# StephenNG59/ICP-symm

Hardware: AMD Instinct MI355X
Metric: icp_iterations_per_sec (higher is better)
Workload: dtype f32

## Files before the change

icp-symm_amd/csrc/engine.cpp:

```cpp
#include "engine_internal.h"
#include "robust_loss.h"
#include <limits>

void read_switches(Switches &w)
{
    auto flag = [](const char *n) { return std::getenv(n) != nullptr; };
    auto num = [](const char *n, long def) { const char *e = std::getenv(n); return e ? std::atol(e) : def; };
    auto tri = [](const char *n) { const char *e = std::getenv(n); return e ? (e[0] == '1' ? 1 : 0) : -1; };
    w.allow_any_arch = flag("SYMMICP_ALLOW_ANY_ARCH");
    w.debug_host = flag("SYMMICP_DEBUG_HOST");
    w.debug_counters = flag("SYMMICP_DEBUG_COUNTERS");
    if (const char *e = std::getenv("SYMMICP_DEBUG_TRACE")) w.debug_trace = e;
    if (const char *e = std::getenv("SYMMICP_GRID_PPC")) w.grid_ppc = std::atof(e);
    w.grid_maxlevel = (int)num("SYMMICP_GRID_MAXLEVEL", kMortonBits);
    w.grid_level = (int)num("SYMMICP_GRID_LEVEL", -1);
    if (const char *e = std::getenv("SYMMICP_FIRST_PASS")) w.first_pass = (e[0] == 'p') ? 1 : 0;
    w.oct_leaf = (int)num("SYMMICP_OCT_LEAF", 0);
    if (const char *e = std::getenv("SYMMICP_PACKET_ORDER")) w.packet_order = e[0] != '0';
    if (const char *e = std::getenv("SYMMICP_PACKET_JUMP")) w.packet_jump = (float)std::atof(e);
    w.packet_key_bits = (int)num("SYMMICP_PACKET_KEY_BITS", 16);
    w.packet_chunk = (uint32_t)num("SYMMICP_PACKET_CHUNK", 0);
    w.packet_lds_pad = (uint32_t)num("SYMMICP_PACKET_LDS_PAD", 0);
    w.packet_waves = (uint32_t)num("SYMMICP_PACKET_WAVES", 0);
    w.packet_front_cap = (uint32_t)num("SYMMICP_PACKET_FRONT_CAP", 0);
    if (const char *e = std::getenv("SYMMICP_HOOD_FRAC")) w.hood_frac = std::atof(e);
    w.no_hood = flag("SYMMICP_NO_NEIGHBOURHOOD");
    w.no_cert = flag("SYMMICP_NO_CERT");
    w.walk_full_grid = flag("SYMMICP_WALK_FULL_GRID");
    { const char *e = std::getenv("SYMMICP_HOST_LOOP"); w.host_loop = e && e[0] == '1'; }
    w.no_loop_stragglers = flag("SYMMICP_NO_LOOP_STRAGGLERS");
    w.force_comm = flag("SYMMICP_FORCE_COMM");
    if (const char *e = std::getenv("SYMMICP_PACKET_COST_KEY")) w.packet_cost_key = e[0] != '0';
    w.budget_walk = tri("SYMMICP_BUDGET_WALK");
    w.optimistic = tri("SYMMICP_OPTIMISTIC");
    w.compact = tri("SYMMICP_COMPACT");
    w.cert_pass = (int)num("SYMMICP_CERT_PASS", 1);
    w.cert_head = (int)num("SYMMICP_CERT_HEAD", 4);
    w.pass_blocks = (int)num("SYMMICP_PASS_BLOCKS", 2048);
    w.id_blocks = (int)num("SYMMICP_ID_BLOCKS", 2048);
    w.acc_blocks = (int)num("SYMMICP_ACC_BLOCKS", 512);
    w.fused_blocks = (int)num("SYMMICP_FUSED_BLOCKS", 512);
    w.compact_blocks = (int)num("SYMMICP_COMPACT_BLOCKS", 1280);
    w.feature_nn_splits = (int)num("SYMMICP_FEATURE_NN_SPLITS", 0);
    w.feature_nn_queries = (int)num("SYMMICP_FEATURE_NN_QUERIES", 0);
    w.plane_score = (int)num("SYMMICP_PLANE_SCORE", 0);
    w.tune.wave_mode_max =(uint32_t)num("SYMMICP_WAVE_MODE_MAX", 20000);
    w.tune.cells_chunk = (uint32_t)num("SYMMICP_CELLS_CHUNK", 16);
    w.tune.cells_queries = (uint32_t)num("SYMMICP_CELLS_QUERIES", 0);
    w.tune.walk_budget = (uint32_t)num("SYMMICP_WALK_BUDGET", 160);
}

void arena_begin(Arena &a, size_t want)
{
    a.off = 0;
    if (a.cap >= want) return;
    if (a.base) hipFree(a.base);
    a.base = nullptr; a.cap = 0;
    const size_t cap = want + want / 4;
    if (hipMalloc((void **)&a.base, cap) == hipSuccess) a.cap = cap;
    else (void)hipGetLastError();
// ... 1108 lines not shown
```

icp-symm_amd/csrc/engine_debug.cpp:

```cpp
#include "engine_internal.h"

static constexpr size_t kTraceWords = (size_t)1 << 22;
void dump_packet_trace(symmicp_ctx *c)
{
    if (FILE *f = std::fopen(c->sw.debug_trace.c_str(), "wb")) {
        std::vector<unsigned long long> t(kTraceWords);
        hipMemcpy(t.data(), c->dbg_trace, t.size() * 8, hipMemcpyDeviceToHost);
        std::fwrite(t.data(), 8, t.size(), f);
        std::fclose(f);
    }
    hipMemset(c->dbg_trace, 0, kTraceWords * 8);
}


void print_pass_counters(symmicp_ctx *c, bool first, long long list_len)
{
        unsigned long long h[12];
        hipMemcpy(h, c->ix.dbg, sizeof(h), hipMemcpyDeviceToHost);
        hipMemset(c->ix.dbg, 0, sizeof(h));
        if (first && c->cfg.corr == SYMMICP_CORR_TREE && c->target_surface_like)
            std::fprintf(stderr, "[symmicp dbg] pass %lld (packets): steps=%llu nodes+leaf candidates=%llu leaf candidates rejected=%llu points=%llu tie rescans=%llu overflows=%llu lanes wanting a scanned leaf (sum)=%llu | packet ticks (10 ns): sum=%llu max=%llu\n",
                         (long long)c->st.passes, h[0], h[4], h[5], h[3], h[2], h[1], h[8], h[7], h[6]);
        else
        std::fprintf(stderr, "[symmicp dbg] pass %lld: cells: certified=%llu (by neighbourhood %llu) scans=%llu (neighbourhoods kept %llu, not kept %llu) probes=%llu to-walk=%llu items=%llu points=%llu | walk list=%lld visits=%llu wave-max*64=%llu\n",
                     (long long)c->st.passes, h[1], h[8], h[2], h[9], h[10], h[6], h[7], h[0], h[3], list_len, h[4], h[5]);
}

void print_batch_summary(const symmicp_ctx *c, int it0, int it1, int want, int enq, int n_stage, const uint8_t *pass_kernel, const PassFeedback &before)
{
    const bool tree = c->cfg.corr == SYMMICP_CORR_TREE;
    auto list_of = [](const PassFeedback &f) { return f.list_known() ? (long long)f.list_len : (f.expects_list() ? -2ll : -1ll); };
    if (it1 - it0 >= 2) {
        const double *q = ring_at(c, it1 - 1).sums;
        if (q[37] != 0.0) std::fprintf(stderr, "[symmicp host] k_reduce_solve stamps of pass %d: load + reduce %.2f us (loop state there after %.2f us), bookkeeping + solve %.2f us, publish %.2f us\n", it1 - 1, std::floor(q[37]) * 0.01, (q[37] - std::floor(q[37])) * 1e4 * 0.01, q[38] * 0.01, q[39] * 0.01);
    }
    int n_cert = 0;
    for (int k = it0 + 1; k <= it1; k++) n_cert += pass_kernel[ring_slot(k)];
    if (tree) {
        std::fprintf(stderr, "[symmicp host] batch: work list / searched pairs / scanned pairs after each device pass (c: certified-only kernel):");
        for (int k = it0 + 1; k <= it1; k++) {
            const LoopRecord &r = ring_at(c, k);
            std::fprintf(stderr, " %d/%d/%d%s", r.list_len, r.searched, r.scans, pass_kernel[ring_slot(k)] ? "c" : "");
        }
        std::fprintf(stderr, "\n");
    }
    std::fprintf(stderr, "[symmicp host] batch: %d of %d passes on the device (%d enqueued), reason %d, %d with the straggler stage, %d certified-only%s, list after %lld (host pass before: list %lld, scanned %lld)\n", it1 - it0, want, enq, c->h_loop->reason, n_stage, n_cert, c->cert_pass_failed ? " (now off: a pass came back incomplete)" : "", list_of(c->fb), list_of(before), before.counts_known() ? (long long)before.scans : -1ll);
}
```

icp-symm_amd/csrc/engine_internal.h:

```cpp
#pragma once
#include <hip/hip_runtime.h>
#include <dlfcn.h>
#include <fcntl.h>
#include <sys/mman.h>
#include <sys/stat.h>
#include <unistd.h>
#include <algorithm>
#include <chrono>
#include <cmath>
#include <cstdio>
#include <cstdlib>
#include <cstring>
#include <limits>
#include <mutex>
#include <string>
#include <vector>

#include "symmicp.h"
#include "symmicp_internal.h"
#include "host_solve.h"
#include "loop_plan.h"


namespace symmicp {}
// ... 38 lines not shown
};
extern Rccl g_rccl;

inline double now_s()
{
    return std::chrono::duration<double>(std::chrono::steady_clock::now().time_since_epoch()).count();
}

struct Switches {
    bool allow_any_arch = false, debug_host = false, debug_counters = false;
    std::string debug_trace;
    double grid_ppc = 3.0;
    int grid_maxlevel = kMortonBits, grid_level = -1;
    int first_pass = -1;
    int oct_leaf = 0;
    bool packet_order = true;
    bool packet_cost_key = true;
    float packet_jump = -1.0f;
    int packet_key_bits = 16;
    uint32_t packet_chunk = 0, packet_lds_pad = 0, packet_waves = 0, packet_front_cap = 0;
    double hood_frac = 0.8;
    bool no_hood = false, no_cert = false, walk_full_grid = false, host_loop = false, no_loop_stragglers = false, force_comm = false;
    int budget_walk = -1, optimistic = -1, compact = -1;
    int cert_pass = 1;
    int cert_head = 4;
    int pass_blocks = 2048, id_blocks = 2048, acc_blocks = 512, fused_blocks = 512, compact_blocks = 1280;
    int feature_nn_splits = 0, feature_nn_queries = 0;
    int plane_score = 0;
    PassTuning tune;
};

void read_switches(Switches &w);

struct Arena {
    char *base = nullptr;
    size_t cap = 0, off = 0;
};

struct ShmSlot {
    volatile unsigned long long seq;
    double s[SYMMICP_NSUM];
    char pad[512 - 8 - 8 * SYMMICP_NSUM];
};
static_assert(sizeof(ShmSlot) == 512, "slot = 4 cache lines");
struct ShmExchange {
    ShmSlot *slots = nullptr;
    size_t bytes = 0;
    unsigned long long count = 0;
// ... 281 lines not shown
```

icp-symm_amd/csrc/engine_loop.cpp:

```cpp
#include "engine_internal.h"

extern "C" {

static int prepare_rejectors(symmicp_ctx *c, RejectArgs &r)
{
    Rejectors &j = c->rej;
    r = RejectArgs{};
    if (!pass_rejects(c)) return SYMMICP_OK;
    HIP_TRY(c, grow(j.keys, j.keys_cap, c->n_loc ? c->n_loc : 1));
    if (!j.ws) HIP_TRY(c, hipMalloc((void **)&j.ws, sizeof(uint32_t) * kRejectWsWords));
    r.keys = j.keys; r.ws = j.ws;
    r.host = reinterpret_cast<RejectRecord *>(c->h_sums_dev + kNSum + 1);
    r.rho = j.trim_frac; r.med_f2 = j.median() ? j.med_factor * j.med_factor : 0.0f;
    if (!pass_claims(c)) return SYMMICP_OK;
    HIP_TRY(c, grow(j.table, j.table_cap, Rejectors::table_words(c->n_t, pass_reciprocal(c))));
    r.table = j.table; r.n_t = c->n_t; r.order = c->src_order;
    r.claim = kClaimOneToOne;
    if (!pass_reciprocal(c)) return SYMMICP_OK;
    if (!j.src_ix.valid) {
        const double t0 = now_s();
        if (int st = build_reverse_index(c, c->src0, c->n_loc, c->src_order, j.src_ix)) return st;
        j.src_ix_builds++;
        if (c->sw.debug_host) {
            std::fprintf(stderr, "[symmicp host] source index: %u points, %zu bytes in its arena (+%zu allocations beside it), built in %.3f ms\n", c->n_loc,
// ... 248 lines not shown
    return batch_eligible(in);
}

static constexpr int kListBlocks = 8;
static constexpr int kEvSampleStride = 4;

struct BatchRun {
    LoopConfig lc;
    PassArgs a;
    ChunkPlanner planner;
    bool tree, vec4;
    bool timed;
    int ev_stride;
    int want, it0;
    int blocks_full;
    uint32_t *counters;
    int enq, n_stage;
    uint8_t pass_kernel[symmicp_ctx::kRing];
    symmicp_sums last0;
    PassFeedback fb0;
};
struct Chunk {
    int nq, it_before, ev_used0;
    bool certified, stage;
    int fused_blocks, blocks;
};

static LoopConfig make_loop_config(const symmicp_ctx *c, int want)
{
    LoopConfig lc{};
    lc.mode = c->cfg.mode; lc.fixed_iters = c->cfg.fixed_iters; lc.max_iters = c->iters + want;
    lc.incremental = resolved_apply(c->cfg) == SYMMICP_APPLY_INCREMENTAL ? 1 : 0; lc.tree = c->cfg.corr == SYMMICP_CORR_TREE ? 1 : 0;
    lc.diff_threshold = c->cfg.diff_threshold; lc.eps_rotation = c->cfg.eps_rotation; lc.eps_translation = c->cfg.eps_translation;
    lc.nrm_w = (c->cfg.mode == SYMMICP_MODE_QUIRKS) ? 1.0f : 0.0f;
    for (int k = 0; k < 3; k++) lc.pivot[k] = c->pivot[k];
    lc.uncertified_limit = loop_slow_limit(c->n_s_total);
    lc.list_limit = kLoopListLimit;
    if (lc.max_iters > c->cfg.max_iters) lc.max_iters = c->cfg.max_iters;
    return lc;
}

static int begin_batch(symmicp_ctx *c, BatchRun &run, int want)
{
    const bool incr = resolved_apply(c->cfg) == SYMMICP_APPLY_INCREMENTAL;
    run.tree = c->cfg.corr == SYMMICP_CORR_TREE;
    run.want = want; run.it0 = c->iters; run.fb0 = c->fb;
    run.lc = make_loop_config(c, want);
    const int cert_mode = (run.tree && c->cert && !c->sw.no_cert && !c->cert_pass_failed) ? c->sw.cert_pass : 0;
    const bool one_piece = run.lc.fixed_iters && !(run.lc.eps_rotation > 0.f && run.lc.eps_translation > 0.f);
    run.planner = ChunkPlanner(run.tree && !c->sw.no_loop_stragglers, c->fb.has_list(), cert_mode, one_piece, c->sw.cert_head);
    LoopState ls{};
    std::memcpy(ls.X, c->X, sizeof(ls.X));
    for (int k = 0; k < 12; k++) ls.Xapply.m[k] = c->X[k];
    ls.Xapply.nrm_w = run.lc.nrm_w;
    ls.iters = run.it0;
    *c->h_loop = ls;
    if (c->loop_log_on) {
        run.last0 = c->last;
        ring_at(c, run.it0).solved = 0;
    }
    HIP_TRY(c, hipMemcpyAsync(c->d_loop, c->h_loop, sizeof(LoopState), hipMemcpyHostToDevice, c->stream));
    fill_pass_args(c, run.a, RejectArgs{}, plan_pass(c, false, incr), c->X, incr, incr, false);
    run.a.loop = c->d_loop;
    if (run.tree) run.blocks_full = fused_pass_blocks(c->n_loc, c->sw.fused_blocks);
    else {
        const IdentityGrid g = identity_grid(c->n_loc, c->n_t, c->src_off, c->sw.id_blocks);
        run.blocks_full = g.blocks; run.vec4 = g.vec4;
    }
    c->pass_blocks = run.blocks_full;
    run.counters = run.tree ? c->wl_count : nullptr;
    run.timed = c->timing == 1 || c->timing == 3;
    run.ev_stride = c->timing == 3 ? kEvSampleStride : 1;
    if (run.timed && c->ev_used + want > symmicp_ctx::kEvRing) flush_events(c);
    return SYMMICP_OK;
}

static Chunk begin_chunk(symmicp_ctx *c, BatchRun &run, const ChunkPlan &plan)
{
    Chunk ch{};
    ch.nq = (run.want - run.enq < plan.passes) ? run.want - run.enq : plan.passes;
    ch.it_before = c->h_loop->iters;
    ch.ev_used0 = c->ev_used;
    ch.certified = plan.certified;
    ch.stage = run.planner.stragglers();
    ch.fused_blocks = (ch.stage && run.blocks_full + kListBlocks > 512) ? 512 - kListBlocks : run.blocks_full;
    ch.blocks = ch.fused_blocks + (ch.stage ? kListBlocks : 0);
    run.a.partial_cols = ch.stage ? (uint32_t)ch.blocks : 0u;
    run.a.partial_col0 = (uint32_t)ch.fused_blocks;
    run.lc.walk_in_loop = ch.stage ? 1 : 0;
    return ch;
}

static int enqueue_pass(symmicp_ctx *c, BatchRun &run, const Chunk &ch, int p)
{
    hipEvent_t *ev = nullptr;
    if (run.timed && (run.enq + p) % run.ev_stride == 0 && c->ev_used < symmicp_ctx::kEvRing) {
        ev = c->ev + c->ev_used * symmicp_ctx::kEvPer;
        c->ev_split[c->ev_used] = 1;
        c->ev_weight[c->ev_used] = 1;
        hipEventRecord(ev[0], c->stream);
    }
    if (run.tree) {
        run.pass_kernel[ring_slot(ch.it_before + 1 + p)] = ch.certified ? 1 : 0;
        if (ch.certified) launch_pass_certified(run.a, c->ix, c->wl, ch.fused_blocks, c->stream);
        else launch_pass_fused(run.a, c->ix, c->wl, ch.fused_blocks, c->stream);
        if (ch.stage) launch_loop_stragglers(run.a, c->ix, c->wl, kListBlocks, c->sw.tune, c->stream);
    }
    else launch_pass_identity(run.a, c->tgt, ch.blocks, run.vec4, c->stream);
    if (ev) { hipEventRecord(ev[4], c->stream); c->ev_used++; }
    if (!(c->comm || ch.blocks > 512)) {
        launch_reduce_solve(c->partials, ch.blocks, c->d_sums, 0, c->d_loop, run.lc, c->h_ring_dev, symmicp_ctx::kRing, run.counters, c->stream);
        return SYMMICP_OK;
    }
    launch_final_reduce(c->partials, ch.blocks, c->d_sums, nullptr, c->ticket, 0ull, run.counters, 0, c->stream);
    if (c->comm) {
        if (ev) { hipEventRecord(ev[6], c->stream); c->ev_coll[c->ev_used - 1] = 1; }
        if (int st = allreduce_record(c)) {
            (void)hipStreamSynchronize(c->stream);
            c->begun = false;
            c->ev_used = 0;
            return st;
        }
        if (ev) hipEventRecord(ev[7], c->stream);
    }
    launch_reduce_solve(c->partials, ch.blocks, c->d_sums, 1, c->d_loop, run.lc, c->h_ring_dev, symmicp_ctx::kRing, run.counters, c->stream);
    return SYMMICP_OK;
}
// ... 44 lines not shown
    if (redo && run.pass_kernel[ring_slot(it1 + 1)]) c->cert_pass_failed = true;
    if (c->sw.debug_host) print_batch_summary(c, it0, it1, run.want, run.enq, run.n_stage, run.pass_kernel, run.fb0);
    if (hl.reason == LOOP_SLOW) c->host_passes_since_bailout = 1;
    if (redo || hl.reason == LOOP_HOST_SOLVE) {
        c->host_passes_since_bailout = 0;
        c->fb.forget_list();
        c->st.kernel_launches[7]++;
    }
    return SYMMICP_OK;
}

static void append_loop_log(symmicp_ctx *c, const BatchRun &run)
{
    const LoopState &hl = *c->h_loop;
    const int it0 = run.it0, it1 = hl.iters;
    for (int k = it0; k <= it1; k++) {
        const LoopRecord &r = ring_at(c, k);
        symmicp_loop_log_entry e{};
        std::memcpy(e.sums, k == it0 ? run.last0.s : r.sums, sizeof(e.sums));
        std::memcpy(e.increment, r.increment, sizeof(e.increment));
        std::memcpy(e.X, r.X, sizeof(e.X));
        e.rcond = r.rcond; e.iter = k; e.status = r.status; e.solved = r.solved; e.list_len = k == it0 ? 0 : r.list_len;
        e.reason = hl.reason; e.batch = c->loop_log_batches;
        e.reserved = k == it0 ? 0 : run.pass_kernel[ring_slot(k)];
        if (k == it1 && hl.reason == LOOP_REDO_PASS && run.pass_kernel[ring_slot(it1 + 1)]) e.reserved |= 0x100;
        if (!e.solved) { std::memset(e.increment, 0, sizeof(e.increment)); std::memset(e.X, 0, sizeof(e.X)); e.rcond = 0.f; e.status = -1; }
        c->loop_log.push_back(e);
    }
    c->loop_log_batches++;
}

static int run_batch(symmicp_ctx *c, int want, float *diffs_before, int *n_done, bool *small_step)
{
    *n_done = 0;
    *small_step = false;
    if (want > symmicp_ctx::kRing - 1) want = symmicp_ctx::kRing - 1;
    if (want <= 0) return SYMMICP_OK;
    BatchRun run{};
    if (int st = begin_batch(c, run, want)) return st;
    ChunkPlan plan = run.planner.next(c->fb.list_len, c->fb.scans, want, 0);
    while (run.enq < want) {
        const Chunk ch = begin_chunk(c, run, plan);
        if (run.enq == 0) launch_reduce_solve(c->partials, ch.blocks, c->d_sums, 2, c->d_loop, run.lc, c->h_ring_dev, symmicp_ctx::kRing, run.counters, c->stream);
        for (int p = 0; p < ch.nq; p++)
            if (int st = enqueue_pass(c, run, ch, p)) return st;
        if (int st = close_chunk(c, run, ch)) return st;
        if (c->h_loop->stop) break;
// ... 312 lines not shown
```

icp-symm_amd/csrc/kernels_pass.hip:

```cpp
#include <cstdlib>
#include <type_traits>
#include "symmicp_internal.h"
#include "device_common.h"
#include "oct_walk.h"
#include "solve_core.h"
#include "loop_plan.h"
#include "robust_loss.h"
#include "pass_rows.h"
#pragma clang fp contract(off)

namespace symmicp {

template <int NA>
__device__ __forceinline__ void acc_block_reduce_store(AccN<NA> &a, double *partials, uint32_t col)
{
    __shared__ double red[(kPassThreads / 64) * kNSum];
    acc_wave_reduce(a, red + (threadIdx.x >> 6) * kNSum);
    __syncthreads();
    if (threadIdx.x < kNSum) {
        double s = 0.0;
        if (threadIdx.x < NA) {
#pragma unroll
            for (int w = 0; w < kPassThreads / 64; w++) s += red[w * kNSum + threadIdx.x];
        }
// ... 751 lines not shown
            since = 0;
            __syncthreads();
            if (s_cnt > (uint32_t)(kList - kCheck * (int)kTilePts)) flush();
        }
    }
    __syncthreads();
    flush();
    if (threadIdx.x == 0 && s_total) atomicAdd(wl.work.counts + shard * kShardStride + 1, s_total);
    if (ACC && threadIdx.x == 0 && s_hood) atomicAdd(wl.work.counts + shard * kShardStride + 3, s_hood);
#ifdef RS_STAMPS2
    const unsigned long long fs2 = __builtin_amdgcn_s_memrealtime();
#endif
    if (ACC) acc_block_reduce_store(acc, a.partials, blockIdx.x);
#ifdef RS_STAMPS2
    if (ACC && blockIdx.x == 0 && threadIdx.x == 0) {
        double *dbg = a.partials + (size_t)8191 * kNSum;
        dbg[0] = (double)(fs1 - fs0); dbg[1] = (double)(fs2 - fs1); dbg[2] = (double)(__builtin_amdgcn_s_memrealtime() - fs2);
    }
#endif
}

constexpr uint32_t kCertList = kPassThreads;

template <bool W, int OBJ>
__global__ __launch_bounds__(kPassThreads) void k_pass_certified(PassArgs a, TargetIndex ix, WorkLists wl)
{
    const bool need_n = reads_src_normals<OBJ>(false, a.min_ndot);
    __shared__ uint32_t s_list[kCertList];
    __shared__ uint32_t s_cnt, s_bad;
    AccT<W> acc; acc_zero(acc);
    if (threadIdx.x == 0) { s_cnt = 0; s_bad = 0; }
    __syncthreads();
    int stop = 0;
    HotParams h = hot_params(a);
    if (a.loop) {
        stop = a.loop->stop;
        const float4 *xp = reinterpret_cast<const float4 *>(&in_vgpr(a.loop)->Xapply);
        const float4 r0 = xp[0], r1 = xp[1], r2 = xp[2];
        h.X.m[0] = r0.x; h.X.m[1] = r0.y; h.X.m[2] = r0.z; h.X.m[3] = r0.w;
        h.X.m[4] = r1.x; h.X.m[5] = r1.y; h.X.m[6] = r1.z; h.X.m[7] = r1.w;
        h.X.m[8] = r2.x; h.X.m[9] = r2.y; h.X.m[10] = r2.z; h.X.m[11] = r2.w;
        h.X.nrm_w = reinterpret_cast<const float *>(xp)[12];
    }
    const Affine &X = h.X;
    const uint32_t tiles = (a.n + kPassThreads - 1) / kPassThreads;
    const uint32_t tiles_p = ((tiles + 7u) / 8u) * 8u;
    for (uint32_t t = blockIdx.x; t < tiles_p; t += gridDim.x) {
        const uint32_t i = xcd_remap(t, tiles_p) * kPassThreads + threadIdx.x;
        const bool live = i < a.n;
        float x = 0.f, y = 0.f, z = 0.f, nx = 0.f, ny = 0.f, nz = 0.f;
        float4 q = make_float4(0.f, 0.f, 0.f, 0.f), nq = make_float4(0.f, 0.f, 0.f, 2.0f), ce = make_float4(0.f, 0.f, 0.f, 0.f);
        if (live) {
            x = a.in.x[i]; y = a.in.y[i]; z = a.in.z[i];
            if (need_n) { nx = a.in.nx[i]; ny = a.in.ny[i]; nz = a.in.nz[i]; }
            q = a.pairrec[2 * (size_t)i]; nq = a.pairrec[2 * (size_t)i + 1];
            ce = a.cert[i];
        }
        if (stop) return;
        if (!live) continue;
        const float px = xf_row(X.m + 0, x, y, z, 1.0f), py = xf_row(X.m + 4, x, y, z, 1.0f), pz = xf_row(X.m + 8, x, y, z, 1.0f);
        bool certified = false;
        float d2 = 0.0f;
        if (nq.w == 0.0f) {
            d2 = dist2(px, py, pz, q.x, q.y, q.z);
            const float m2 = dist2(px, py, pz, ce.x, ce.y, ce.z);
            certified = (__builtin_amdgcn_sqrtf(d2) + __builtin_amdgcn_sqrtf(m2)) * 1.000002f < ce.w;
        }
        if (certified) pair_step<OBJ>(acc, h, nx, ny, nz, px, py, pz, q, nq, d2);
        else {
            const uint32_t e = atomicAdd(&s_cnt, 1u);
            if (e < kCertList) s_list[e] = i;
        }
    }
    __syncthreads();
    const uint32_t cnt = s_cnt;
    if (cnt) {
        const uint32_t m = min(cnt, kCertList);
        if (threadIdx.x < m) {
            const uint32_t i = s_list[threadIdx.x];
            bool settled = false;
            const float4 ce = a.cert[i];
            const float4 q = a.pairrec[2 * (size_t)i], nq = a.pairrec[2 * (size_t)i + 1];
            const int32_t pk = a.pos_prev[i];
            const float x = a.in.x[i], y = a.in.y[i], z = a.in.z[i];
            float nx = 0.0f, ny = 0.0f, nz = 0.0f;
            if (need_n) { nx = a.in.nx[i]; ny = a.in.ny[i]; nz = a.in.nz[i]; }
            uint4 w0 = make_uint4(kHoodNone, kHoodNone, kHoodNone, kHoodNone), w1 = w0;
            float T = 0.0f;
            if (a.certk) { w0 = a.certk[2 * (size_t)i]; w1 = a.certk[2 * (size_t)i + 1]; T = a.hoodr[i].x; }
            if (a.certk && (__float_as_uint(ce.w) & 1u)) {
                if (nq.w == 0.0f && (uint32_t)pk < ix.n) {
                    const float px = xf_row(X.m + 0, x, y, z, 1.0f), py = xf_row(X.m + 4, x, y, z, 1.0f), pz = xf_row(X.m + 8, x, y, z, 1.0f);
                    const float d2 = dist2(px, py, pz, q.x, q.y, q.z);
                    int32_t pw; float d2w;
                    if (d2 <= __int_as_float(0x7f800000) &&
                        hood_test_set(a, ix, i, px, py, pz, dist2(px, py, pz, ce.x, ce.y, ce.z), pk, d2, __float_as_int(q.w), w0, w1, T, pw, d2w)) {
                        float4 qw = q, nqw = nq;
                        if (pw != pk) { qw = ix.tn[2 * (size_t)pw]; nqw = ix.tn[2 * (size_t)pw + 1]; }
                        pair_step<OBJ>(acc, h, nx, ny, nz, px, py, pz, qw, nqw, d2w);
                        settled = true;
                    }
                }
            }
            if (!settled) atomicAdd(&s_bad, 1u);
        }
        __syncthreads();
        if (threadIdx.x == 0) {
            const uint32_t shard = blockIdx.x & (kShards - 1);
            const uint32_t bad = s_bad + (cnt - m);
            if (bad) atomicAdd(wl.work.counts + shard * kShardStride, bad);
            atomicAdd(wl.work.counts + shard * kShardStride + 1, cnt);
            atomicAdd(wl.work.counts + shard * kShardStride + 3, cnt - bad);
        }
    }
    acc_block_reduce_store(acc, a.partials, blockIdx.x);
}


__device__ __forceinline__ float boxmaxdist2(float px, float py, float pz, const float4 &lo, const float4 &hi)
{
    float dx = fmaxf(fabsf(px - lo.x), fabsf(px - hi.x));
    float dy = fmaxf(fabsf(py - lo.y), fabsf(py - hi.y));
    float dz = fmaxf(fabsf(pz - lo.z), fabsf(pz - hi.z));
    return (dx * dx + dy * dy) + dz * dz;
}

__device__ __forceinline__ unsigned long long wave_min_u64(unsigned long long v)
{
#pragma unroll
    for (int off = 32; off > 0; off >>= 1) {
        unsigned long long o = __shfl_xor(v, off, 64);
        v = o < v ? o : v;
    }
    return v;
}
// ... 631 lines not shown
            hipLaunchKernelGGL(k_search_walk<true>, dim3(walk_blocks), dim3(kWalkThreads), 0, s, a, ix, wl, wl.work, wmm, budget);
            hipLaunchKernelGGL(k_search_walk<false>, dim3(8192), dim3(kWalkThreads), 0, s, a, ix, wl, wl.retry, 0xFFFFFFFFu, 0xFFFFFFFFu);
        } else {
            hipLaunchKernelGGL(k_search_walk<false>, dim3(walk_blocks), dim3(kWalkThreads), 0, s, a, ix, wl, wl.work, wmm, 0xFFFFFFFFu);
        }
    }
    if (ev) hipEventRecord(ev[3], s);
    launch_accumulate(a, ix.tn, acc_blocks, s);
    if (ev) hipEventRecord(ev[4], s);
}

void launch_final_reduce(const double *partials, int blocks, double *out_dev, double *out_host_mapped, uint32_t *ticket,
                         unsigned long long seq, uint32_t *counters_to_clear, int keep_nonempty, hipStream_t s)
{
    hipLaunchKernelGGL(k_final_reduce, dim3(kNSum), dim3(256), 0, s, partials, blocks, out_dev, out_host_mapped, ticket, seq,
                       counters_to_clear, keep_nonempty);
}

void launch_pass_fused(const PassArgs &a, const TargetIndex &ix, const WorkLists &wl, int blocks, hipStream_t s)
{
    with_instantiation(a, [&](auto W, auto OBJ) { hipLaunchKernelGGL((k_pass_fused<true, W, OBJ>), dim3(blocks), dim3(kPassThreads), 0, s, a, ix, wl); });
}

void launch_pass_certified(const PassArgs &a, const TargetIndex &ix, const WorkLists &wl, int blocks, hipStream_t s)
{
    with_instantiation(a, [&](auto W, auto OBJ) { hipLaunchKernelGGL((k_pass_certified<W, OBJ>), dim3(blocks), dim3(kPassThreads), 0, s, a, ix, wl); });
}

void launch_loop_stragglers(const PassArgs &a, const TargetIndex &ix, const WorkLists &wl, int list_blocks, const PassTuning &tune, hipStream_t s)
{
    const uint32_t wave_mode_max = tune.wave_mode_max;
    hipLaunchKernelGGL(k_search_walk<false>, dim3(512), dim3(kWalkThreads), 0, s, a, ix, wl, wl.work, wave_mode_max, 0xFFFFFFFFu);
    with_instantiation(a, [&](auto W, auto OBJ) {
        hipLaunchKernelGGL((k_accumulate_list<W, OBJ>), dim3(list_blocks), dim3(kPassThreads), 0, s, a, ix.tn, wl.work);
    });
}

void launch_reduce_solve(const double *partials, int blocks, double *out_dev, int mode, LoopState *loop, LoopConfig cfg, LoopRecord *ring, int ring_len,
                         uint32_t *counters_to_clear, hipStream_t s)
{
    if (mode == 0) hipLaunchKernelGGL(k_reduce_solve<true>, dim3(1), dim3(512), 0, s, partials, blocks, out_dev, 0, loop, cfg, ring, ring_len, counters_to_clear);
    else hipLaunchKernelGGL(k_reduce_solve<false>, dim3(1), dim3(512), 0, s, partials, blocks, out_dev, mode == 2 ? 1 : 0, loop, cfg, ring, ring_len, counters_to_clear);
}

void launch_loop_end(const LoopState *loop, LoopState *host_copy, unsigned long long *done_flag, unsigned long long seq, hipStream_t s)
{
    hipLaunchKernelGGL(k_loop_end, dim3(1), dim3(64), 0, s, loop, host_copy, done_flag, seq);
}

// ... 23 lines not shown
```

icp-symm_amd/csrc/loop_plan.h:

```cpp
#pragma once
#include <math.h>
#include <stdint.h>
#include "symmicp.h"

#if defined(__HIPCC__) || defined(__CUDACC__)
#define LOOP_PLAN_HD __host__ __device__
#else
#define LOOP_PLAN_HD
#endif

namespace symmicp {

struct PassFeedback {
    enum class List : uint8_t { kUnknown, kKnown, kExpected };
    List list = List::kUnknown;
    bool counts = false;
    uint64_t list_len = 0;
    uint64_t searched = 0, scans = 0;

    bool list_known() const { return list == List::kKnown; }
    bool list_empty() const { return list_known() && list_len == 0; }
    bool has_list() const { return list_known() && list_len > 0; }
    bool expects_list() const { return list == List::kExpected; }
    bool counts_known() const { return counts; }
// ... 81 lines not shown
{
    TreePassPlan p{};
    p.acc_blocks = accumulate_blocks(in.n_loc, in.acc_blocks);
    if (!in.first && in.fb.list_known() && in.fb.list_len <= kWalkSizedListMax) {
        p.walk_blocks = (uint32_t)(2 * in.fb.list_len);
        if (p.walk_blocks < 256u) p.walk_blocks = 256u;
        if (p.walk_blocks > 8192u) p.walk_blocks = 8192u;
    }
    if (!in.first && in.fb.expects_list()) p.walk_blocks = 16384u;
    if (in.walk_full_grid) p.walk_blocks = 0;
    p.optimistic = in.optimistic >= 0 ? in.optimistic == 1 : (!in.first && in.fb.list_empty());
    if (in.writeback) p.optimistic = false;
    if (in.rejecting) p.optimistic = false;
    const bool compact = in.use_slack && (in.compact >= 0 ? in.compact == 1 : (in.fb.counts_known() && in.fb.searched < (uint64_t)(in.n_s_total / 10)));
    p.compact_blocks = compact ? in.compact_blocks : 0;
    p.make_hood = in.have_certk && !in.first && in.fb.counts_known() && (double)in.fb.searched < in.hood_frac * (double)in.n_s_total;
    p.budget_walk = in.budget_walk >= 0 ? in.budget_walk != 0 : (in.first && in.nranks > 1 && in.n_loc < 400000u);
    return p;
}

constexpr uint32_t kLoopListLimit = 8192;
inline uint32_t loop_scan_limit(uint32_t n) { const uint32_t f = n / 256; return f < 8192u ? f : 8192u; }
inline uint32_t loop_slow_limit(uint32_t n) { return 4 * loop_scan_limit(n); }

struct BatchEligibleIn {
    bool host_loop_switch;
    bool rejecting;
    bool color;
    bool host_loop_config;
    bool host_exchange;
    bool host_diagnostics;
    bool device_solves;
    bool empty_share_alone;
    int host_passes_since_bailout;
    bool identity, tree;
    bool incremental;
    bool certificates;
    bool no_loop_stragglers;
    uint32_t n_s_total;
    PassFeedback fb;
};
inline bool batch_eligible(const BatchEligibleIn &in)
{
    if (in.host_loop_switch) return false;
    if (in.rejecting) return false;
    if (in.color) return false;
    if (in.host_loop_config) return false;
    if (in.host_exchange) return false;
    if (in.host_diagnostics) return false;
    if (!in.device_solves) return false;
    if (in.empty_share_alone) return false;
    if (in.host_passes_since_bailout < 2) return false;
    if (in.identity) return true;
    if (in.tree)
        return !in.incremental && in.fb.list_known() && in.fb.list_len <= (in.no_loop_stragglers ? 0u : kLoopListLimit) && in.fb.counts_known() &&
               in.fb.searched <= loop_scan_limit(in.n_s_total) / (in.fb.list_len > 0 ? 2u : 1u) && in.certificates;
    return false;
}

struct ChunkPlan {
    int passes;
    bool certified;
};
class ChunkPlanner {
public:
    static constexpr int kCertHeads = 3;
    ChunkPlanner() = default;
    ChunkPlanner(bool stage_allowed, bool list_at_entry, int cert_mode, bool one_piece, int cert_head)
        : cert_mode_(cert_mode), cert_head_(cert_head), stage_allowed_(stage_allowed), one_piece_(one_piece)
    {
        set_stage(list_at_entry);
        heads_left_ = (one_piece_ && !stragglers_ && cert_mode_ == 1 && cert_head_ > 0) ? kCertHeads : 0;
    }
    bool stragglers() const { return stragglers_; }
    ChunkPlan next(uint64_t list_len, uint64_t scans, int left, int prev)
    {
        const bool certified = cert_mode_ == 2 || (cert_mode_ == 1 && !stragglers_ && list_len == 0 && scans == 0);
        if (stragglers_) return ChunkPlan{4, certified};
        if (!one_piece_) return ChunkPlan{prev ? 2 * prev : 4, certified};
        if (!certified && heads_left_ > 0 && left > cert_head_) { heads_left_--; return ChunkPlan{cert_head_, certified}; }
        return ChunkPlan{left, certified};
    }
    void after_chunk(bool any_list_in_chunk) { set_stage(any_list_in_chunk); }

private:
    void set_stage(bool on) { stragglers_ = stage_allowed_ && on && cert_mode_ != 2; }
    int cert_mode_ = 0, cert_head_ = 0, heads_left_ = 0;
    bool stage_allowed_ = false, one_piece_ = false, stragglers_ = false;
};

}
```

icp-symm_amd/csrc/symmicp_internal.h:

```cpp
#pragma once
#include <hip/hip_runtime.h>
#include <stdint.h>
#include <stddef.h>
#include "symmicp.h"

namespace symmicp {

constexpr int kNSum = SYMMICP_NSUM;
constexpr int kNAcc = 37;
constexpr int kNAccW = 38;
constexpr int kLeaf = 8;
constexpr int kFan = 8;
constexpr int kMaxTreeLevels = 12;
constexpr int kMortonBits = 10;
constexpr int kPassThreads = 256;
constexpr int kBruteTile = 1024;
constexpr int kBruteQ = 4;

constexpr bool mode_device_solves(int mode)
{
    return mode == SYMMICP_MODE_QUIRKS || mode == SYMMICP_MODE_PAPER || mode == SYMMICP_MODE_PLANE || mode == SYMMICP_MODE_GICP;
}
constexpr bool mode_known(int mode)
{
// ... 118 lines not shown
    float max_d2;
    float min_ndot;
    int32_t p2p;
    int32_t writeback;
    const unsigned long long *best64;
    int32_t *pos_prev;
    float *d2_out;
    int32_t *pos_out;
    double *partials;
    float4 *pairrec;
    int32_t budget_walk;
    int32_t refresh_records;
    float4 *cert;
    uint4 *certk;
    float2 *hoodr;
    int32_t make_hood;
    int32_t use_slack;
    const LoopState *loop;
    uint32_t partial_cols, partial_col0;
    const uint2 *pkt_tab;
    uint32_t pkt_count;
    uint32_t pkt_waves;
    uint32_t pkt_front_cap;
    uint32_t *pkt_fallbacks;
    uint32_t pkt_chunk, pkt_lds_pad;
    int32_t loss;
    float loss_scale;
    int32_t obj;
    float gicp_k;
    RejectArgs rej;
    const float4 *tgt_color;
    const float *src_int;
    float color_lam, color_om;
};
static_assert(sizeof(PassArgs) == 432 && offsetof(PassArgs, rej) == 344 && offsetof(PassArgs, tgt_color) == 408 && offsetof(PassArgs, src_int) == 416,
              "PassArgs keeps its layout");
__host__ __device__ inline bool pass_rejects(const PassArgs &a) { return a.rej.keys != nullptr; }

struct PassTuning {
    uint32_t wave_mode_max = 20000u;
    uint32_t cells_chunk = 16u;
    uint32_t cells_queries = 0u;
    uint32_t walk_budget = 160u;
};

constexpr int kBatchThreads = 512;
// ... 10 lines not shown
};
struct BatchArgs {
    const float *src_xyz, *src_nrm, *tgt_xyz, *tgt_nrm;
    const BatchProblem *problems;
    const float *guess;
    symmicp_batch_result *out;
    float *trace_X;
    double *trace_sums;
    int32_t mode, max_iters, fixed_iters;
    float diff_threshold, max_d2, min_ndot, eps_rotation, eps_translation;
};
void launch_batch_align(const BatchArgs &a, uint32_t n_problems, hipStream_t s);

void launch_pass_identity(const PassArgs &a, CloudSoA tgt, int blocks, bool vec4_ok, hipStream_t s);
void launch_pass_indexed(const PassArgs &a, const float4 *tn , int blocks, hipStream_t s);
void launch_pass_tree_split(const PassArgs &a, const TargetIndex &ix, const WorkLists &wl, int acc_blocks, uint32_t walk_blocks,
                            int stage, int compact_blocks, const PassTuning &tune, hipStream_t s, hipEvent_t *ev);
void launch_pass_tree_first(const PassArgs &a, const TargetIndex &ix, const WorkLists &wl, int acc_blocks, hipStream_t s, hipEvent_t *ev);
uint32_t walk_blocks_full(const WorkLists &wl);
uint32_t shard_capacity(uint32_t n_points);
void launch_final_reduce(const double *partials, int blocks, double *out_dev, double *out_host_mapped, uint32_t *ticket,
                         unsigned long long seq, uint32_t *counters_to_clear, int keep_nonempty, hipStream_t s);
void launch_pass_fused(const PassArgs &a, const TargetIndex &ix, const WorkLists &wl, int blocks, hipStream_t s);
void launch_pass_certified(const PassArgs &a, const TargetIndex &ix, const WorkLists &wl, int blocks, hipStream_t s);
void launch_loop_stragglers(const PassArgs &a, const TargetIndex &ix, const WorkLists &wl, int list_blocks, const PassTuning &tune, hipStream_t s);
void launch_reduce_solve(const double *partials, int blocks, double *out_dev, int mode, LoopState *loop, LoopConfig cfg, LoopRecord *ring, int ring_len,
                         uint32_t *counters_to_clear, hipStream_t s);
void launch_solve_probe(int mode, int exact_rc, const symmicp_sums *sums, int n, const float *pivot, const float *X_in, int32_t *status, float *pbar,
                        float *qbar, float *a, float *t, float *rcond, float *out16, float *X_out, hipStream_t s);
void launch_loop_end(const LoopState *loop, LoopState *host_copy, unsigned long long *done_flag, unsigned long long seq, hipStream_t s);
void launch_publish(const double *sums_dev, double *out_host_mapped, unsigned long long seq, hipStream_t s);
void launch_nn_brute(const CloudSoA &src, uint32_t n_s, const Affine &X, const float4 *tq, uint32_t n_t,
                     unsigned long long *best64, hipStream_t s);

void launch_bbox(const float *x, const float *y, const float *z, uint32_t n, uint32_t *bbox_ord6, hipStream_t s);
void launch_morton(const float *x, const float *y, const float *z, uint32_t n, float ox, float oy, float oz,
                   float inv_h0, uint32_t *keys, uint32_t *vals, hipStream_t s);
void radix_sort_pairs(uint32_t *keys, uint32_t *vals, uint32_t *keys_tmp, uint32_t *vals_tmp, uint32_t n,
                      int key_bits, uint32_t *hist_ws, size_t hist_ws_elems, hipStream_t s);
size_t radix_sort_ws_elems(uint32_t n);
void launch_gather_f4(const float *x, const float *y, const float *z, const float *nx, const float *ny, const float *nz,
                      const uint32_t *order, uint32_t n, float4 *tq, float4 *tn, hipStream_t s);
void launch_gather_soa(const CloudSoA &src, const uint32_t *order, uint32_t n, CloudSoA dst, hipStream_t s);
void launch_offset_u32(const uint32_t *in, uint32_t off, uint32_t n, uint32_t *out, hipStream_t s);
void launch_packet_runs(const CloudSoA &src, uint32_t n, float jump_factor, uint2 *runs, uint32_t *keys, uint32_t *vals, uint32_t *count, int key_bits, hipStream_t s);
void launch_packet_cost(const CloudSoA &src, const uint2 *runs, uint32_t npk, const TargetIndex &ix, uint32_t *keys, int key_bits, hipStream_t s);
void launch_packet_table(const uint32_t *order, const uint2 *runs, uint32_t npk, uint2 *tab, hipStream_t s);
// ... 184 lines not shown
```

icp-symm_amd/py/symmicp/__init__.py:

```python
import ctypes as C
import os
import sys

import numpy as np

_PKG = os.path.dirname(os.path.abspath(__file__))
_ROOT = os.path.dirname(os.path.dirname(_PKG))
LIB_PATH = os.environ.get("SYMMICP_LIB") or os.path.join(_ROOT, "lib", "libsymmicp.so")

NSUM = 40
UNIQUE_ID_BYTES = 128
OK, ERR_ARG, ERR_SIZE, ERR_DEGENERATE, ERR_IO, ERR_HIP, ERR_STATE, ERR_COMM = range(8)
ERR_NO_CONSENSUS = 8
RANSAC_EVALUATED, RANSAC_REPEATED, RANSAC_EDGE, RANSAC_DEGENERATE, RANSAC_FAR = range(5)
PLANE_EVALUATED, PLANE_REPEATED, PLANE_DEGENERATE, PLANE_OFF_AXIS = range(4)
MODE_QUIRKS, MODE_PAPER, MODE_P2P, MODE_PLANE, MODE_GICP, MODE_COLOR, MODE_NDT = 0, 1, 2, 3, 5, 7, 9
CORR_IDENTITY, CORR_BRUTE, CORR_TREE = 0, 1, 2
APPLY_DEFAULT, APPLY_INCREMENTAL, APPLY_CUMULATIVE = 0, 1, 2
LOSS_NONE, LOSS_HUBER, LOSS_TUKEY, LOSS_CAUCHY, LOSS_GEMAN_MCCLURE = range(5)
_LOSS_NAMES = {"none": LOSS_NONE, "huber": LOSS_HUBER, "tukey": LOSS_TUKEY, "cauchy": LOSS_CAUCHY,
               "geman_mcclure": LOSS_GEMAN_MCCLURE}

_STATUS_NAMES = {0: "OK", 1: "ERR_ARG", 2: "ERR_SIZE", 3: "ERR_DEGENERATE", 4: "ERR_IO", 5: "ERR_HIP",
                 6: "ERR_STATE", 7: "ERR_COMM", 8: "ERR_NO_CONSENSUS"}
# ... 1952 lines not shown
    def reciprocal_info(self):
        v, b, n, t = C.c_int32(0), C.c_uint64(0), C.c_uint64(0), C.c_uint64(0)
        self._chk(self._L.symmicp_ctx_reciprocal_info(self._h, C.byref(v), C.byref(b), C.byref(n), C.byref(t)))
        return dict(index_valid=bool(v.value), index_bytes=b.value, index_builds=n.value, table_words=t.value)

    def scan_probe(self, data):
        d = np.array(data, np.uint32).reshape(-1)
        self._chk(self._L.symmicp_ctx_scan_probe(self._h, d.ctypes.data_as(C.POINTER(C.c_uint32)), d.size))
        return d

    def set_loop_log(self, on=True):
        self._chk(self._L.symmicp_set_loop_log(self._h, int(bool(on))))

    def loop_log(self):
        n = C.c_size_t(0)
        self._chk(self._L.symmicp_get_loop_log(self._h, None, 0, C.byref(n)))
        buf = (LoopLogEntry * max(1, n.value))()
        self._chk(self._L.symmicp_get_loop_log(self._h, buf, n.value, C.byref(n)))
        out = []
        for e in buf[:n.value]:
            out.append(dict(sums=np.array(e.sums[:], np.float64), increment=np.array(e.increment[:], np.float32).reshape(4, 4),
                            X=np.array(e.X[:], np.float32).reshape(4, 4), rcond=e.rcond, iter=e.iter, status=e.status, solved=e.solved,
                            list_len=e.list_len, reason=e.reason, batch=e.batch,
                            kernel=e.reserved & 0xff, redo_certified=bool(e.reserved & 0x100)))
        return out


class MyICP:

    def __init__(self, mode=MODE_QUIRKS, corr=CORR_IDENTITY, max_iters=10, diff_threshold=1.0, verbose=True, **extra):
        self._cfg = dict(mode=mode, corr=corr, max_iters=max_iters, diff_threshold=diff_threshold,
                         verbose=int(bool(verbose)), **extra)
        self.cloud_src = self.cloud_tgt = None
        self.normals_src = self.normals_tgt = None
        self._final = np.eye(4, dtype=np.float32)
        self.last_result = None
        self._loss = (LOSS_NONE, 0.0)
        self._gicp_eps = None
        self._trim = 1.0
        self._one_to_one = False
        self._reciprocal = False
        self._median = 0.0
        self._color_weight = None
        self.intensity_src = self.intensity_tgt = None
        self._levels = []
        self._ndt = dict(resolution=1.0, neighbors=7, min_points=6)
        self._ndt_levels = []
# ... 379 lines not shown
```

Baseline: 33590.

## Let certified-only pass resolve a small scan tail in-kernel

```diff
diff --git a/icp-symm_amd/csrc/engine.cpp b/icp-symm_amd/csrc/engine.cpp
--- a/icp-symm_amd/csrc/engine.cpp
+++ b/icp-symm_amd/csrc/engine.cpp
@@ -34,8 +34,11 @@
     w.budget_walk = tri("SYMMICP_BUDGET_WALK");
     w.optimistic = tri("SYMMICP_OPTIMISTIC");
     w.compact = tri("SYMMICP_COMPACT");
-    w.cert_pass = (int)num("SYMMICP_CERT_PASS", 1);
+    w.cert_pass = (int)num("SYMMICP_CERT_PASS", 3);
     w.cert_head = (int)num("SYMMICP_CERT_HEAD", 4);
+    w.cert_tail = num("SYMMICP_CERT_TAIL", -1);
+    w.cert_list = (int)num("SYMMICP_CERT_LIST", 256);
+    if (w.cert_list < 1 || w.cert_list > 256) w.cert_list = 256;
     w.pass_blocks = (int)num("SYMMICP_PASS_BLOCKS", 2048);
     w.id_blocks = (int)num("SYMMICP_ID_BLOCKS", 2048);
     w.acc_blocks = (int)num("SYMMICP_ACC_BLOCKS", 512);
diff --git a/icp-symm_amd/csrc/engine_debug.cpp b/icp-symm_amd/csrc/engine_debug.cpp
--- a/icp-symm_amd/csrc/engine_debug.cpp
+++ b/icp-symm_amd/csrc/engine_debug.cpp
@@ -34,15 +34,15 @@
         const double *q = ring_at(c, it1 - 1).sums;
         if (q[37] != 0.0) std::fprintf(stderr, "[symmicp host] k_reduce_solve stamps of pass %d: load + reduce %.2f us (loop state there after %.2f us), bookkeeping + solve %.2f us, publish %.2f us\n", it1 - 1, std::floor(q[37]) * 0.01, (q[37] - std::floor(q[37])) * 1e4 * 0.01, q[38] * 0.01, q[39] * 0.01);
     }
-    int n_cert = 0;
-    for (int k = it0 + 1; k <= it1; k++) n_cert += pass_kernel[ring_slot(k)];
+    int n_cert = 0, n_tail = 0;
+    for (int k = it0 + 1; k <= it1; k++) { n_cert += pass_kernel[ring_slot(k)] & 1; n_tail += (pass_kernel[ring_slot(k)] >> 1) & 1; }
     if (tree) {
-        std::fprintf(stderr, "[symmicp host] batch: work list / searched pairs / scanned pairs after each device pass (c: certified-only kernel):");
+        std::fprintf(stderr, "[symmicp host] batch: work list / searched pairs / scanned pairs after each device pass (c: certified-only kernel, t: with its scan tail):");
         for (int k = it0 + 1; k <= it1; k++) {
             const LoopRecord &r = ring_at(c, k);
-            std::fprintf(stderr, " %d/%d/%d%s", r.list_len, r.searched, r.scans, pass_kernel[ring_slot(k)] ? "c" : "");
+            std::fprintf(stderr, " %d/%d/%d%s", r.list_len, r.searched, r.scans, (pass_kernel[ring_slot(k)] & 2) ? "t" : (pass_kernel[ring_slot(k)] ? "c" : ""));
         }
         std::fprintf(stderr, "\n");
     }
-    std::fprintf(stderr, "[symmicp host] batch: %d of %d passes on the device (%d enqueued), reason %d, %d with the straggler stage, %d certified-only%s, list after %lld (host pass before: list %lld, scanned %lld)\n", it1 - it0, want, enq, c->h_loop->reason, n_stage, n_cert, c->cert_pass_failed ? " (now off: a pass came back incomplete)" : "", list_of(c->fb), list_of(before), before.counts_known() ? (long long)before.scans : -1ll);
+    std::fprintf(stderr, "[symmicp host] batch: %d of %d passes on the device (%d enqueued), reason %d, %d with the straggler stage, %d certified-only (%d with the scan tail)%s, list after %lld (host pass before: list %lld, scanned %lld)\n", it1 - it0, want, enq, c->h_loop->reason, n_stage, n_cert, n_tail, c->cert_pass_failed ? " (now off: a pass came back incomplete)" : "", list_of(c->fb), list_of(before), before.counts_known() ? (long long)before.scans : -1ll);
 }
diff --git a/icp-symm_amd/csrc/engine_internal.h b/icp-symm_amd/csrc/engine_internal.h
--- a/icp-symm_amd/csrc/engine_internal.h
+++ b/icp-symm_amd/csrc/engine_internal.h
@@ -84,8 +84,10 @@
     double hood_frac = 0.8;
     bool no_hood = false, no_cert = false, walk_full_grid = false, host_loop = false, no_loop_stragglers = false, force_comm = false;
     int budget_walk = -1, optimistic = -1, compact = -1;
-    int cert_pass = 1;
+    int cert_pass = 3;
     int cert_head = 4;
+    long cert_tail = -1;
+    int cert_list = 256;
     int pass_blocks = 2048, id_blocks = 2048, acc_blocks = 512, fused_blocks = 512, compact_blocks = 1280;
     int feature_nn_splits = 0, feature_nn_queries = 0;
     int plane_score = 0;
diff --git a/icp-symm_amd/csrc/engine_loop.cpp b/icp-symm_amd/csrc/engine_loop.cpp
--- a/icp-symm_amd/csrc/engine_loop.cpp
+++ b/icp-symm_amd/csrc/engine_loop.cpp
@@ -294,7 +294,7 @@
 };
 struct Chunk {
     int nq, it_before, ev_used0;
-    bool certified, stage;
+    bool certified, tail, stage;
     int fused_blocks, blocks;
 };
 
@@ -320,7 +320,8 @@
     run.lc = make_loop_config(c, want);
     const int cert_mode = (run.tree && c->cert && !c->sw.no_cert && !c->cert_pass_failed) ? c->sw.cert_pass : 0;
     const bool one_piece = run.lc.fixed_iters && !(run.lc.eps_rotation > 0.f && run.lc.eps_translation > 0.f);
-    run.planner = ChunkPlanner(run.tree && !c->sw.no_loop_stragglers, c->fb.has_list(), cert_mode, one_piece, c->sw.cert_head);
+    const uint64_t tail_scans = cert_tail_scans(c->n_s_total / (uint32_t)(c->nranks > 0 ? c->nranks : 1), c->sw.cert_tail);
+    run.planner = ChunkPlanner(run.tree && !c->sw.no_loop_stragglers, c->fb.has_list(), cert_mode, one_piece, c->sw.cert_head, tail_scans);
     LoopState ls{};
     std::memcpy(ls.X, c->X, sizeof(ls.X));
     for (int k = 0; k < 12; k++) ls.Xapply.m[k] = c->X[k];
@@ -334,6 +335,7 @@
     HIP_TRY(c, hipMemcpyAsync(c->d_loop, c->h_loop, sizeof(LoopState), hipMemcpyHostToDevice, c->stream));
     fill_pass_args(c, run.a, RejectArgs{}, plan_pass(c, false, incr), c->X, incr, incr, false);
     run.a.loop = c->d_loop;
+    run.a.cert_list_cap = (uint32_t)c->sw.cert_list;
     if (run.tree) run.blocks_full = fused_pass_blocks(c->n_loc, c->sw.fused_blocks);
     else {
         const IdentityGrid g = identity_grid(c->n_loc, c->n_t, c->src_off, c->sw.id_blocks);
@@ -354,6 +356,7 @@
     ch.it_before = c->h_loop->iters;
     ch.ev_used0 = c->ev_used;
     ch.certified = plan.certified;
+    ch.tail = plan.certified && plan.tail;
     ch.stage = run.planner.stragglers();
     ch.fused_blocks = (ch.stage && run.blocks_full + kListBlocks > 512) ? 512 - kListBlocks : run.blocks_full;
     ch.blocks = ch.fused_blocks + (ch.stage ? kListBlocks : 0);
@@ -373,8 +376,8 @@
         hipEventRecord(ev[0], c->stream);
     }
     if (run.tree) {
-        run.pass_kernel[ring_slot(ch.it_before + 1 + p)] = ch.certified ? 1 : 0;
-        if (ch.certified) launch_pass_certified(run.a, c->ix, c->wl, ch.fused_blocks, c->stream);
+        run.pass_kernel[ring_slot(ch.it_before + 1 + p)] = ch.certified ? (ch.tail ? 3 : 1) : 0;
+        if (ch.certified) launch_pass_certified(run.a, c->ix, c->wl, ch.fused_blocks, ch.tail, c->stream);
         else launch_pass_fused(run.a, c->ix, c->wl, ch.fused_blocks, c->stream);
         if (ch.stage) launch_loop_stragglers(run.a, c->ix, c->wl, kListBlocks, c->sw.tune, c->stream);
     }
@@ -465,7 +468,8 @@
         std::memcpy(e.X, r.X, sizeof(e.X));
         e.rcond = r.rcond; e.iter = k; e.status = r.status; e.solved = r.solved; e.list_len = k == it0 ? 0 : r.list_len;
         e.reason = hl.reason; e.batch = c->loop_log_batches;
-        e.reserved = k == it0 ? 0 : run.pass_kernel[ring_slot(k)];
+        e.reserved = k == it0 ? 0 : (run.pass_kernel[ring_slot(k)] & 1);
+        if (k != it0 && r.scans > 0) e.reserved |= (r.scans < 0x7fff ? r.scans : 0x7fff) << 16;
         if (k == it1 && hl.reason == LOOP_REDO_PASS && run.pass_kernel[ring_slot(it1 + 1)]) e.reserved |= 0x100;
         if (!e.solved) { std::memset(e.increment, 0, sizeof(e.increment)); std::memset(e.X, 0, sizeof(e.X)); e.rcond = 0.f; e.status = -1; }
         c->loop_log.push_back(e);
diff --git a/icp-symm_amd/csrc/kernels_pass.hip b/icp-symm_amd/csrc/kernels_pass.hip
--- a/icp-symm_amd/csrc/kernels_pass.hip
+++ b/icp-symm_amd/csrc/kernels_pass.hip
@@ -797,12 +797,13 @@
 
 constexpr uint32_t kCertList = kPassThreads;
 
-template <bool W, int OBJ>
-__global__ __launch_bounds__(kPassThreads) void k_pass_certified(PassArgs a, TargetIndex ix, WorkLists wl)
+template <bool W, int OBJ, bool TAIL>
+__global__ __launch_bounds__(kPassThreads, TAIL ? 2 : 1) void k_pass_certified(PassArgs a, TargetIndex ix, WorkLists wl)
 {
     const bool need_n = reads_src_normals<OBJ>(false, a.min_ndot);
     __shared__ uint32_t s_list[kCertList];
     __shared__ uint32_t s_cnt, s_bad;
+    const uint32_t cap = TAIL ? ((a.cert_list_cap - 1u < kCertList) ? a.cert_list_cap : kCertList) : kCertList;
     AccT<W> acc; acc_zero(acc);
     if (threadIdx.x == 0) { s_cnt = 0; s_bad = 0; }
     __syncthreads();
@@ -844,13 +845,14 @@
         if (certified) pair_step<OBJ>(acc, h, nx, ny, nz, px, py, pz, q, nq, d2);
         else {
             const uint32_t e = atomicAdd(&s_cnt, 1u);
-            if (e < kCertList) s_list[e] = i;
+            if (e < cap) s_list[e] = i;
         }
     }
     __syncthreads();
     const uint32_t cnt = s_cnt;
     if (cnt) {
-        const uint32_t m = min(cnt, kCertList);
+        const uint32_t m = min(cnt, cap);
+        uint32_t mine = 0xFFFFFFFFu;
         if (threadIdx.x < m) {
             const uint32_t i = s_list[threadIdx.x];
             bool settled = false;
@@ -877,15 +879,32 @@
                     }
                 }
             }
-            if (!settled) atomicAdd(&s_bad, 1u);
+            if (!settled) { atomicAdd(&s_bad, 1u); if (TAIL) mine = i; }
         }
         __syncthreads();
+        const uint32_t shard = blockIdx.x & (kShards - 1);
+        const uint32_t unsettled = s_bad;
+        const bool scan = TAIL && unsettled && cnt == m;
+        if (scan) {
+            cells_tile<true>(a, ix, wl, X, mine, shard, true);
+            __syncthreads();
+            if (mine != 0xFFFFFFFFu) {
+                const uint32_t i = mine;
+                const float4 q = a.pairrec[2 * (size_t)i], nq = a.pairrec[2 * (size_t)i + 1];
+                if (nq.w == 0.0f) {
+                    const float x = a.in.x[i], y = a.in.y[i], z = a.in.z[i];
+                    float nx = 0.0f, ny = 0.0f, nz = 0.0f;
+                    if (need_n) { nx = a.in.nx[i]; ny = a.in.ny[i]; nz = a.in.nz[i]; }
+                    const float px = xf_row(X.m + 0, x, y, z, 1.0f), py = xf_row(X.m + 4, x, y, z, 1.0f), pz = xf_row(X.m + 8, x, y, z, 1.0f);
+                    pair_step<OBJ>(acc, h, nx, ny, nz, px, py, pz, q, nq, dist2(px, py, pz, q.x, q.y, q.z));
+                }
+            }
+        }
         if (threadIdx.x == 0) {
-            const uint32_t shard = blockIdx.x & (kShards - 1);
-            const uint32_t bad = s_bad + (cnt - m);
+            const uint32_t bad = (scan ? 0u : unsettled) + (cnt - m);
             if (bad) atomicAdd(wl.work.counts + shard * kShardStride, bad);
             atomicAdd(wl.work.counts + shard * kShardStride + 1, cnt);
-            atomicAdd(wl.work.counts + shard * kShardStride + 3, cnt - bad);
+            atomicAdd(wl.work.counts + shard * kShardStride + 3, TAIL ? m - unsettled : cnt - bad);
         }
     }
     acc_block_reduce_store(acc, a.partials, blockIdx.x);
@@ -1563,9 +1582,12 @@
     with_instantiation(a, [&](auto W, auto OBJ) { hipLaunchKernelGGL((k_pass_fused<true, W, OBJ>), dim3(blocks), dim3(kPassThreads), 0, s, a, ix, wl); });
 }
 
-void launch_pass_certified(const PassArgs &a, const TargetIndex &ix, const WorkLists &wl, int blocks, hipStream_t s)
-{
-    with_instantiation(a, [&](auto W, auto OBJ) { hipLaunchKernelGGL((k_pass_certified<W, OBJ>), dim3(blocks), dim3(kPassThreads), 0, s, a, ix, wl); });
+void launch_pass_certified(const PassArgs &a, const TargetIndex &ix, const WorkLists &wl, int blocks, bool tail, hipStream_t s)
+{
+    with_instantiation(a, [&](auto W, auto OBJ) {
+        if (tail) hipLaunchKernelGGL((k_pass_certified<W, OBJ, true>), dim3(blocks), dim3(kPassThreads), 0, s, a, ix, wl);
+        else hipLaunchKernelGGL((k_pass_certified<W, OBJ, false>), dim3(blocks), dim3(kPassThreads), 0, s, a, ix, wl);
+    });
 }
 
 void launch_loop_stragglers(const PassArgs &a, const TargetIndex &ix, const WorkLists &wl, int list_blocks, const PassTuning &tune, hipStream_t s)
diff --git a/icp-symm_amd/csrc/loop_plan.h b/icp-symm_amd/csrc/loop_plan.h
--- a/icp-symm_amd/csrc/loop_plan.h
+++ b/icp-symm_amd/csrc/loop_plan.h
@@ -127,6 +127,12 @@
 constexpr uint32_t kLoopListLimit = 8192;
 inline uint32_t loop_scan_limit(uint32_t n) { const uint32_t f = n / 256; return f < 8192u ? f : 8192u; }
 inline uint32_t loop_slow_limit(uint32_t n) { return 4 * loop_scan_limit(n); }
+constexpr uint32_t kTailMinShare = 65536u, kTailDivisor = 1024u;
+inline uint64_t cert_tail_scans(uint32_t share, long forced)
+{
+    if (forced >= 0) return (uint64_t)forced;
+    return share < kTailMinShare ? 0u : (uint64_t)(share / kTailDivisor);
+}
 
 struct BatchEligibleIn {
     bool host_loop_switch;
@@ -166,13 +172,15 @@
 struct ChunkPlan {
     int passes;
     bool certified;
+    bool tail = false;
 };
 class ChunkPlanner {
 public:
     static constexpr int kCertHeads = 3;
     ChunkPlanner() = default;
-    ChunkPlanner(bool stage_allowed, bool list_at_entry, int cert_mode, bool one_piece, int cert_head)
-        : cert_mode_(cert_mode), cert_head_(cert_head), stage_allowed_(stage_allowed), one_piece_(one_piece)
+    ChunkPlanner(bool stage_allowed, bool list_at_entry, int cert_mode, bool one_piece, int cert_head, uint64_t tail_scans = 0)
+        : tail_scans_(cert_mode == 3 ? tail_scans : 0), cert_mode_(cert_mode == 3 ? 1 : cert_mode), cert_head_(cert_head),
+          stage_allowed_(stage_allowed), one_piece_(one_piece)
     {
         set_stage(list_at_entry);
         heads_left_ = (one_piece_ && !stragglers_ && cert_mode_ == 1 && cert_head_ > 0) ? kCertHeads : 0;
@@ -180,16 +188,19 @@
     bool stragglers() const { return stragglers_; }
     ChunkPlan next(uint64_t list_len, uint64_t scans, int left, int prev)
     {
-        const bool certified = cert_mode_ == 2 || (cert_mode_ == 1 && !stragglers_ && list_len == 0 && scans == 0);
-        if (stragglers_) return ChunkPlan{4, certified};
-        if (!one_piece_) return ChunkPlan{prev ? 2 * prev : 4, certified};
-        if (!certified && heads_left_ > 0 && left > cert_head_) { heads_left_--; return ChunkPlan{cert_head_, certified}; }
-        return ChunkPlan{left, certified};
+        const bool tail = tail_scans_ > 0 && cert_mode_ == 1;
+        const bool certified = cert_mode_ == 2 || (cert_mode_ == 1 && !stragglers_ && list_len == 0 && scans <= tail_scans_);
+        const bool t = tail && certified;
+        if (stragglers_) return ChunkPlan{4, certified, t};
+        if (!one_piece_) return ChunkPlan{prev ? 2 * prev : 4, certified, t};
+        if (!certified && heads_left_ > 0 && left > cert_head_) { heads_left_--; return ChunkPlan{cert_head_, certified, t}; }
+        return ChunkPlan{left, certified, t};
     }
     void after_chunk(bool any_list_in_chunk) { set_stage(any_list_in_chunk); }
 
 private:
     void set_stage(bool on) { stragglers_ = stage_allowed_ && on && cert_mode_ != 2; }
+    uint64_t tail_scans_ = 0;
     int cert_mode_ = 0, cert_head_ = 0, heads_left_ = 0;
     bool stage_allowed_ = false, one_piece_ = false, stragglers_ = false;
 };
diff --git a/icp-symm_amd/csrc/symmicp_internal.h b/icp-symm_amd/csrc/symmicp_internal.h
--- a/icp-symm_amd/csrc/symmicp_internal.h
+++ b/icp-symm_amd/csrc/symmicp_internal.h
@@ -164,6 +164,7 @@
     uint32_t pkt_count;
     uint32_t pkt_waves;
     uint32_t pkt_front_cap;
+    uint32_t cert_list_cap;
     uint32_t *pkt_fallbacks;
     uint32_t pkt_chunk, pkt_lds_pad;
     int32_t loss;
@@ -220,7 +221,7 @@
 void launch_final_reduce(const double *partials, int blocks, double *out_dev, double *out_host_mapped, uint32_t *ticket,
                          unsigned long long seq, uint32_t *counters_to_clear, int keep_nonempty, hipStream_t s);
 void launch_pass_fused(const PassArgs &a, const TargetIndex &ix, const WorkLists &wl, int blocks, hipStream_t s);
-void launch_pass_certified(const PassArgs &a, const TargetIndex &ix, const WorkLists &wl, int blocks, hipStream_t s);
+void launch_pass_certified(const PassArgs &a, const TargetIndex &ix, const WorkLists &wl, int blocks, bool tail, hipStream_t s);
 void launch_loop_stragglers(const PassArgs &a, const TargetIndex &ix, const WorkLists &wl, int list_blocks, const PassTuning &tune, hipStream_t s);
 void launch_reduce_solve(const double *partials, int blocks, double *out_dev, int mode, LoopState *loop, LoopConfig cfg, LoopRecord *ring, int ring_len,
                          uint32_t *counters_to_clear, hipStream_t s);
diff --git a/icp-symm_amd/py/symmicp/__init__.py b/icp-symm_amd/py/symmicp/__init__.py
--- a/icp-symm_amd/py/symmicp/__init__.py
+++ b/icp-symm_amd/py/symmicp/__init__.py
@@ -1998,7 +1998,7 @@
             out.append(dict(sums=np.array(e.sums[:], np.float64), increment=np.array(e.increment[:], np.float32).reshape(4, 4),
                             X=np.array(e.X[:], np.float32).reshape(4, 4), rcond=e.rcond, iter=e.iter, status=e.status, solved=e.solved,
                             list_len=e.list_len, reason=e.reason, batch=e.batch,
-                            kernel=e.reserved & 0xff, redo_certified=bool(e.reserved & 0x100)))
+                            kernel=e.reserved & 0xff, redo_certified=bool(e.reserved & 0x100), scans=(e.reserved >> 16) & 0x7fff))
         return out
 
 
```

Result: slower. 33110 (-1.4%).
